# phymhan/pc-gan

Measured on AMD Instinct MI355X. Metric: images/sec (G+D step) 128x128 bs32 per GPU, higher is better.
Workload: dtype f32; 1 GPU; wsgan_emb UTKFace-shaped 128x128 bs32/GPU fp32: 9-block ResnetGenerator + 3-layer PatchGAN + ResNet-18 Elo encoder@224 + AlexNet IP@224, full optimize_parameters(); global_batch=32, parallelism=dp1

## Files before the change

include/pcgan_hip.h:

```cpp
#ifndef PCGAN_HIP_H
#define PCGAN_HIP_H

#include <stddef.h>
#include <stdint.h>

#ifdef __cplusplus
extern "C" {
#endif

typedef void* pcgan_stream_t;

const char* pcgan_last_error(void);
int pcgan_version(void);
int pcgan_device_info(int* cu_count, char* arch, int arch_len);

typedef struct {
    int N, C, H, W;
    int K, R, S;
    int stride, pad, pad_mode;
    int P, Q;
    int dtype;
} pcgan_conv_desc;

enum { PCGAN_ACT_NONE = 0, PCGAN_ACT_RELU = 1, PCGAN_ACT_LRELU = 2, PCGAN_ACT_TANH = 3, PCGAN_ACT_SIGMOID = 4 };
// ... 46 lines not shown
                         int act, float slope, int dtype, pcgan_stream_t s);
int pcgan_bn_bwd_reduce(const float* s1_nc, const float* s2_nc, float* s1_c, float* s2_c, int N, int C,
                        pcgan_stream_t s);
int pcgan_bn_stats_merged(const void* x, float* mean_nc, float* m2_nc, float* mean_c, float* var_c, float* running_mean,
                          float* running_var, long long* batches, unsigned int* ticket, int N, int C, int HW, float momentum, int dtype,
                          pcgan_stream_t s);
int pcgan_bn_bwd_stats_reduced(const void* dy, const void* x, const void* y, const float* mean_c, const float* var_c, float* s1_nc,
                               float* s2_nc, float* s1_c, float* s2_c, unsigned int* ticket, int N, int C, int HW, float eps, int act,
                               float slope, int dtype, pcgan_stream_t s);
int pcgan_bn_fwd_fused(const void* x, const float* gamma, const float* beta, const void* residual, void* y,
                       float* mean_c, float* var_c, float* running_mean, float* running_var, long long* batches, float* y_cmax,
                       int N, int C, int HW, float momentum, float eps, int act, float slope, int dtype, pcgan_stream_t s);
int pcgan_bn_bwd_fused(const void* dy, const void* x, const void* y, const float* mean_c, const float* var_c,
                       const float* gamma, void* dx, void* dres, float* s1_c, float* s2_c, float* dx_cmax, int N, int C, int HW,
                       float eps, int act, float slope, int dtype, pcgan_stream_t s);

int pcgan_instnorm_fwd(const void* x, const void* residual, void* y, float* mean_nc, float* m2_nc, float* y_pmax, int N, int C,
                       int HW, float eps, int act, float slope, int dtype, pcgan_stream_t s);
int pcgan_instnorm_bwd(const void* dy, const void* x, const void* y, const float* mean_nc, const float* m2_nc,
                       void* dx, float* dx_psum, float* dx_pmax, float* ws_s1s2, int N, int C, int HW, float eps, int act,
                       float slope, int dtype, pcgan_stream_t s);
int pcgan_instnorm_fused(int HW);
int pcgan_sum_planes(const float* part_nc, float* out, int N, int C, int accumulate, pcgan_stream_t s);

int pcgan_maxpool_fwd(const void* x, void* y, int32_t* argmax, int NC, int H, int W, int k, int stride,
                      int pad, int P, int Q, int dtype, pcgan_stream_t s);
int pcgan_maxpool_bwd(const void* dy, const int32_t* argmax, void* dx, int NC, int H, int W, int k, int stride,
                      int pad, int P, int Q, int dtype, pcgan_stream_t s);
int pcgan_avgpool_fwd(const void* x, void* y, int NC, int H, int W, int k, int stride, int pad, int P, int Q, int dtype,
                      pcgan_stream_t s);
// ... 223 lines not shown
```

pc-gan_amd/csrc/capi.hip:

```cpp
#include "common.h"
#include <stdarg.h>
#include <atomic>
#include <mutex>
#include <vector>

namespace pcgan {
static thread_local char g_err[512] = "";
void set_error(const char* fmt, ...) {
    va_list ap;
    va_start(ap, fmt);
    vsnprintf(g_err, sizeof(g_err), fmt, ap);
    va_end(ap);
}
}

namespace pcgan {
namespace {
struct TimerKind {
    std::vector<hipEvent_t> start, stop;
    int used = 0;
};
std::mutex g_timer_mu;
std::atomic<int> g_timer_on{0};
TimerKind g_timer[TIMER_KINDS];
// ... 57 lines not shown
    }
    t.used = 0;
    return n;
}

namespace pcgan {
static std::atomic<unsigned*> g_nonfinite{nullptr};
unsigned* nonfinite_counter() { return g_nonfinite.load(std::memory_order_relaxed); }
}
extern "C" int pcgan_set_nonfinite_counter(unsigned int* dev_word) {
    pcgan::g_nonfinite.store(dev_word);
    return 0;
}

namespace pcgan {
static const char* const g_opt_names[OPT_COUNT] = {"bsplit_halo", "wgrad_gen", "wgrad_padcopy", "wgrad_cw", "hgemm_bf16", "wgd_look", "wgrad_direct", "hgemm_tile", "hgemm_ks", "wgrad_rowring", "wgrad_ks", "hwgrad_ks"};
static std::atomic<int> g_opt[OPT_COUNT] = {{1}, {1}, {0}, {0}, {1}, {3}, {0}, {0}, {0}, {1}, {0}, {0}};
int option(int id) { return (id >= 0 && id < OPT_COUNT) ? g_opt[id].load(std::memory_order_relaxed) : 0; }
static int option_index(const char* key) {
    for (int i = 0; key && i < OPT_COUNT; ++i)
        if (strcmp(key, g_opt_names[i]) == 0) return i;
    return -1;
}
}
extern "C" int pcgan_set_option(const char* key, int value) {
    using namespace pcgan;
    const int i = option_index(key);
    PCGAN_CHECK(i >= 0, "set_option: unknown option '%s' (bsplit_halo, wgrad_gen, wgrad_padcopy, wgrad_cw, hgemm_bf16, wgd_look, wgrad_direct, hgemm_tile, hgemm_ks, wgrad_rowring, wgrad_ks, hwgrad_ks)", key ? key : "(null)");
    PCGAN_CHECK(i != OPT_WGRAD_CW || value == 0 || value == 128 || value == 256, "set_option: wgrad_cw takes 0 (default), 128 or 256, got %d", value);
    PCGAN_CHECK(i != OPT_HGEMM_TILE || value == 0 || value == 128128 || value == 128064 || value == 64128 || value == 64064,
                "set_option: hgemm_tile takes 0 (heuristic) or BM * 1000 + BP with BM, BP in {64, 128}, got %d", value);
    PCGAN_CHECK(i != OPT_HGEMM_KS || (value >= 0 && value <= 8), "set_option: hgemm_ks takes 0 (heuristic) .. 8, got %d", value);
    PCGAN_CHECK(i != OPT_WGRAD_KS || (value >= 0 && value <= 512), "set_option: wgrad_ks takes 0 (heuristic) .. 512, got %d", value);
    PCGAN_CHECK(i != OPT_HWGRAD_KS || (value >= 0 && value <= 512), "set_option: hwgrad_ks takes 0 (heuristic) .. 512, got %d", value);
    g_opt[i].store(value);
    return 0;
}
extern "C" int pcgan_get_option(const char* key, int* value) {
    using namespace pcgan;
    const int i = option_index(key);
    PCGAN_CHECK(i >= 0 && value, "get_option: unknown option or null output");
    *value = g_opt[i].load();
    return 0;
}

extern "C" const char* pcgan_last_error(void) { return pcgan::g_err; }
extern "C" int pcgan_version(void) { return 100; }

extern "C" int pcgan_device_info(int* cu_count, char* arch, int arch_len) {
// ... 14 lines not shown
```

pc-gan_amd/csrc/common.h:

```cpp
#pragma once
#include <hip/hip_runtime.h>
#include <stdint.h>
#include <stdio.h>
#include <string.h>
#include "../../include/pcgan_hip.h"

namespace pcgan {

void set_error(const char* fmt, ...);

#define PCGAN_CHECK(cond, ...)                \
    do {                                      \
        if (!(cond)) {                        \
            pcgan::set_error(__VA_ARGS__);    \
            return 1;                         \
        }                                     \
    } while (0)

#define PCGAN_LAUNCH_CHECK()                                                      \
    do {                                                                          \
        hipError_t e__ = hipGetLastError();                                       \
        if (e__ != hipSuccess) {                                                  \
            pcgan::set_error("%s:%d launch failed: %s", __FILE__, __LINE__,       \
                             hipGetErrorString(e__));                             \
// ... 1 lines not shown
        }                                                                         \
    } while (0)

enum { TIMER_RES_FWD = 0, TIMER_RES_DGRAD = 1, TIMER_RES_WGRAD = 2, TIMER_RES_WGRAD_MAIN = 3, TIMER_KINDS = 4 };
struct TimerScope {
    int kind, slot;
    hipStream_t st;
    TimerScope(int kind, hipStream_t st);
    ~TimerScope();
};

static inline int timer_kind_res(const pcgan_conv_desc* d, int kind) {
    return (d && d->K == 256 && d->C == 256 && d->R == 3 && d->S == 3 && d->stride == 1 && d->pad_mode == 1 && d->pad == 1) ? kind : -1;
}

enum { OPT_BSPLIT_HALO = 0, OPT_WGRAD_GEN = 1, OPT_WGRAD_PADCOPY = 2, OPT_WGRAD_CW = 3, OPT_HGEMM_BF16 = 4, OPT_WGD_LOOK = 5, OPT_WGRAD_DIRECT = 6, OPT_HGEMM_TILE = 7, OPT_HGEMM_KS = 8, OPT_WGRAD_ROWRING = 9, OPT_WGRAD_KS = 10, OPT_HWGRAD_KS = 11, OPT_COUNT = 12 };
int option(int id);

unsigned* nonfinite_counter();
int launch_wgd_reduce(const float* part, float* dw, const float* scales, int splits, int K, int C, int accumulate, hipStream_t st);
__device__ __forceinline__ bool is_nonfinite(float v) { return (__float_as_uint(v) & 0x7f800000u) == 0x7f800000u; }
__device__ __forceinline__ void report_nonfinite(unsigned* counter, bool bad) {
    if (counter != nullptr && __builtin_amdgcn_ballot_w64(bad) != 0ull && (threadIdx.x & 63) == 0) atomicAdd(counter, 1u);
}

int launch_weight_row_absmax(const float* w, int K, int C, int T, int by_c, float* out, hipStream_t st);

int launch_reflect_fold(const void* padded, void* dx, int NC, int H, int W, int pad, int dtype, hipStream_t st, const float* bias = nullptr,
                        int C = 1);

static inline int ilog2_exact(int v) {
// ... 176 lines not shown
```

pc-gan_amd/csrc/norm.hip:

```cpp
#include <type_traits>

#include "common.h"

namespace pcgan {

struct BnTicket {
    unsigned* ticket;
    int N, C;
};
template <bool WT>
__device__ __forceinline__ void bn_merge_channel(const float* mean_nc, const float* m2_nc, float* __restrict__ mean_c,
                                                 float* __restrict__ var_c, float* running_mean, float* running_var, int N, int C, int HW,
                                                 float momentum, int c, int lane) {
    float msum = 0.f;
    for (int n = lane; n < N; n += 64) msum += WT ? ld_wt(mean_nc + n * C + c) : mean_nc[n * C + c];
    const float mean = wave_sum(msum) / (float)N;
    float m2 = 0.f;
    for (int n = lane; n < N; n += 64) {
        const float d = (WT ? ld_wt(mean_nc + n * C + c) : mean_nc[n * C + c]) - mean;
        m2 += (WT ? ld_wt(m2_nc + n * C + c) : m2_nc[n * C + c]) + d * d * (float)HW;
    }
    m2 = wave_sum(m2);
    if (lane != 0) return;
    const float cnt = (float)N * (float)HW;
// ... 48 lines not shown
template <int V, bool SQ, typename T>
__device__ __forceinline__ float plane_partial(const T* xp, int n, float mean) {
    float s = 0.f;
    for (int i = threadIdx.x; i < n; i += blockDim.x) {
        float v[V];
        ldv<V>(xp + V * i, v);
        if (SQ) {
#pragma unroll
            for (int e = 0; e < V; ++e) v[e] = (v[e] - mean) * (v[e] - mean);
        }
        s += vsum<V>(v);
    }
    return s;
}

template <typename T>
__global__ void __launch_bounds__(256) plane_stats_kernel(const T* __restrict__ x, float* __restrict__ mean_nc,
                                                          float* __restrict__ m2_nc, int HW, BnTicket tk = BnTicket{nullptr, 0, 0},
                                                          BnMergeOut mo = BnMergeOut{nullptr, nullptr, nullptr, nullptr, nullptr, 0.f}) {
    __shared__ float scratch[16];
    const size_t plane = blockIdx.x;
    const T* xp = x + plane * (size_t)HW;
    const bool v4 = (HW & 3) == 0;
    const float s = v4 ? plane_partial<4, false>(xp, HW >> 2, 0.f) : plane_partial<1, false>(xp, HW, 0.f);
    const float mean = block_sum(s, scratch) / (float)HW;
    const float q = v4 ? plane_partial<4, true>(xp, HW >> 2, mean) : plane_partial<1, true>(xp, HW, mean);
    const float m2 = block_sum(q, scratch);
    if (threadIdx.x == 0) {
        if (tk.ticket != nullptr) {
            st_wt(mean_nc + plane, mean);
            st_wt(m2_nc + plane, m2);
        } else {
            mean_nc[plane] = mean;
            m2_nc[plane] = m2;
        }
    }
    if (tk.ticket != nullptr) {
        __shared__ int last_flag;
        const int c = (int)(plane % (size_t)tk.C);
        if (block_arrives_last(tk.ticket, c, (unsigned)tk.N, &last_flag) && threadIdx.x < 64) {
            bn_merge_channel<true>(mean_nc, m2_nc, mo.mean_c, mo.var_c, mo.running_mean, mo.running_var, tk.N, tk.C, HW, mo.momentum, c, threadIdx.x);
            if (c == 0 && threadIdx.x == 0 && mo.batches) mo.batches[0] += 1;
// ... 84 lines not shown
    const size_t plane = blockIdx.x;
    float mean, rstd, g, b;
    plane_coeffs(a, plane, mean, rstd, g, b);
    const float sc = rstd * g, sh = b - mean * rstd * g;
    const T* xp = (const T*)a.x + plane * (size_t)a.HW;
    const T* rp = a.residual ? (const T*)a.residual + plane * (size_t)a.HW : nullptr;
    T* yp = (T*)a.out + plane * (size_t)a.HW;
    float am = (a.HW & 3) == 0 ? norm_act_plane<4>(a, xp, rp, yp, a.HW >> 2, sc, sh) : norm_act_plane<1>(a, xp, rp, yp, a.HW, sc, sh);
    if (a.pmax) {
        __shared__ float scratch[16];
        am = block_max(am, scratch);
        if (threadIdx.x == 0) a.pmax[plane] = am;
    }
}

template <typename T>
__global__ void __launch_bounds__(256) norm_bwd_stats_kernel(NormArgs a, BnTicket tk = BnTicket{nullptr, 0, 0}, float* s1_c = nullptr,
                                                             float* s2_c = nullptr) {
    __shared__ float scratch[16];
    const size_t plane = blockIdx.x;
    float mean, rstd, g_, b_;
    plane_coeffs(a, plane, mean, rstd, g_, b_);
    const T* xp = (const T*)a.x + plane * (size_t)a.HW;
    const T* dp = (const T*)a.dy + plane * (size_t)a.HW;
    const T* yp = (a.act != PCGAN_ACT_NONE) ? (const T*)a.y + plane * (size_t)a.HW : nullptr;
    float s1 = 0.f, s2 = 0.f;
    for (int i = threadIdx.x; i < a.HW; i += blockDim.x) {
        float g = ld1(dp + i);
        if (yp) g *= act_grad_from_out(ld1(yp + i), a.act, a.slope);
        s1 += g;
        s2 += g * ((ld1(xp + i) - mean) * rstd);
    }
    s1 = block_sum(s1, scratch);
    s2 = block_sum(s2, scratch);
    if (threadIdx.x == 0) {
        if (tk.ticket != nullptr) {
            st_wt((float*)a.out + plane, s1);
            st_wt((float*)a.out2 + plane, s2);
        } else {
            ((float*)a.out)[plane] = s1;
            ((float*)a.out2)[plane] = s2;
        }
    }
    if (tk.ticket != nullptr) {
        __shared__ int last_flag;
        const int c = (int)(plane % (size_t)tk.C);
// ... 150 lines not shown
            float g = d[e];
            if (act != PCGAN_ACT_NONE) g *= act_grad_from_out(yv[e], act, slope);
            gr[e] = g;
            o[e] = kk * (g - m1 - ((xv[e] - mean) * rstd) * m2);
            am = fmaxf(am, fabsf(o[e]));
        }
        if (dx) stv<V>(dx + i, o);
        if (dres) stv<V>(dres + i, gr);
    });
    if (dx && dx_cmax) {
        am = block_max(am, scratch);
        if (threadIdx.x == 0) dx_cmax[c] = am;
    }
}

struct PlaneBlock {
    float* scratch;
    __device__ __forceinline__ int first() const { return threadIdx.x; }
    __device__ __forceinline__ int step() const { return blockDim.x; }
    __device__ __forceinline__ float sum(float v) const { return block_sum(v, scratch); }
    __device__ __forceinline__ float max(float v) const { return block_max(v, scratch); }
};
struct PlaneWave {
    int lane;
    __device__ __forceinline__ int first() const { return lane; }
    __device__ __forceinline__ int step() const { return 64; }
    __device__ __forceinline__ float sum(float v) const { return wave_sum(v); }
    __device__ __forceinline__ float max(float v) const { return wave_max(v); }
};

// ... 214 lines not shown
    static constexpr bool wave = W;
    static constexpr int E = E_;
};
template <typename F>
static void instnorm_dispatch(int E, int NT, int planes, F launch) {
    if (E == 1 && planes >= 1024) launch(InstnormForm<true, 4>{}, dim3((planes + 3) / 4), dim3(256));
    else if (E == 1) launch(InstnormForm<false, 1>{}, dim3(planes), dim3(NT));
    else if (E == 4) launch(InstnormForm<false, 4>{}, dim3(planes), dim3(NT));
    else launch(InstnormForm<false, 16>{}, dim3(planes), dim3(NT));
}
template <typename F>
static void bn_fused_dispatch(int HW, F launch) {
    if ((HW & 3) == 0) launch(std::integral_constant<int, 4>{});
    else launch(std::integral_constant<int, 1>{});
}

}

using namespace pcgan;

extern "C" int pcgan_plane_stats(const void* x, float* mean_nc, float* m2_nc, int NC, int HW, int dtype, pcgan_stream_t s) {
    PCGAN_CHECK(x && mean_nc && m2_nc && NC > 0 && HW > 0, "plane_stats: bad arguments");
    PCGAN_DTYPE_SWITCH(dtype, T, hipLaunchKernelGGL(plane_stats_kernel<T>, dim3(NC), dim3(plane_threads(HW)), 0, (hipStream_t)s,
                                                    (const T*)x, mean_nc, m2_nc, HW));
    PCGAN_LAUNCH_CHECK();
    return 0;
}

extern "C" int pcgan_bn_stats_merged(const void* x, float* mean_nc, float* m2_nc, float* mean_c, float* var_c, float* running_mean,
                                     float* running_var, long long* batches, unsigned int* ticket, int N, int C, int HW, float momentum,
                                     int dtype, pcgan_stream_t s) {
    PCGAN_CHECK(x && mean_nc && m2_nc && mean_c && var_c && ticket && N > 0 && C > 0 && HW > 0 && (long long)N * HW > 1, "bn_stats_merged: bad arguments");
    const BnTicket tk{ticket, N, C};
    const BnMergeOut mo{mean_c, var_c, running_mean, running_var, batches, momentum};
    PCGAN_DTYPE_SWITCH(dtype, T, hipLaunchKernelGGL(plane_stats_kernel<T>, dim3(N * C), dim3(plane_threads(HW)), 0, (hipStream_t)s,
                                                    (const T*)x, mean_nc, m2_nc, HW, tk, mo));
    PCGAN_LAUNCH_CHECK();
    return 0;
}

extern "C" int pcgan_bn_bwd_stats_reduced(const void* dy, const void* x, const void* y, const float* mean_c, const float* var_c, float* s1_nc,
                                          float* s2_nc, float* s1_c, float* s2_c, unsigned int* ticket, int N, int C, int HW, float eps, int act,
                                          float slope, int dtype, pcgan_stream_t s) {
    PCGAN_CHECK(dy && x && mean_c && var_c && s1_nc && s2_nc && s1_c && s2_c && ticket && N > 0 && C > 0 && HW > 0, "bn_bwd_stats_reduced: bad arguments");
    PCGAN_CHECK(act == PCGAN_ACT_NONE || y, "bn_bwd_stats_reduced: activation mask needs y");
    NormArgs a = norm_args(x, mean_c, var_c, N, C, HW, 0, eps, act, slope);
    a.y = y; a.dy = dy; a.out = s1_nc; a.out2 = s2_nc;
    const BnTicket tk{ticket, N, C};
    PCGAN_DTYPE_SWITCH(dtype, T, hipLaunchKernelGGL(norm_bwd_stats_kernel<T>, dim3(N * C), dim3(plane_threads(HW)), 0, (hipStream_t)s, a, tk, s1_c, s2_c));
    PCGAN_LAUNCH_CHECK();
    return 0;
}

extern "C" int pcgan_bn_merge(const float* mean_nc, const float* m2_nc, float* mean_c, float* var_c,
                              float* running_mean, float* running_var, int N, int C, int HW, float momentum,
                              pcgan_stream_t s) {
    PCGAN_CHECK(mean_nc && m2_nc && N > 0 && C > 0 && HW > 0, "bn_merge: bad arguments");
    hipLaunchKernelGGL(bn_merge_kernel, dim3((C + 3) / 4), dim3(256), 0, (hipStream_t)s, mean_nc, m2_nc, mean_c,
                       var_c, running_mean, running_var, N, C, HW, momentum);
    PCGAN_LAUNCH_CHECK();
    return 0;
}

extern "C" int pcgan_in_running_update(const float* mean_nc, const float* m2_nc, float* running_mean,
// ... 13 lines not shown
    PCGAN_CHECK(x && mean && var && y && N > 0 && C > 0 && HW > 0, "norm_act_fwd: bad arguments");
    NormArgs a = norm_args(x, mean, var, N, C, HW, per_plane, eps, act, slope);
    a.gamma = gamma; a.beta = beta; a.residual = residual; a.out = y; a.pmax = y_pmax;
    PCGAN_DTYPE_SWITCH(dtype, T, hipLaunchKernelGGL(norm_act_fwd_kernel<T>, dim3(N * C), dim3(plane_threads(HW)), 0, (hipStream_t)s, a));
    PCGAN_LAUNCH_CHECK();
    return 0;
}

extern "C" int pcgan_norm_bwd_stats(const void* dy, const void* x, const void* y, const float* mean,
                                    const float* var, float* s1_nc, float* s2_nc, int N, int C, int HW,
                                    int per_plane, float eps, int act, float slope, int dtype, pcgan_stream_t s) {
    PCGAN_CHECK(dy && x && mean && var && s1_nc && s2_nc, "norm_bwd_stats: null pointer");
    PCGAN_CHECK(act == PCGAN_ACT_NONE || y, "norm_bwd_stats: activation mask needs y");
    NormArgs a = norm_args(x, mean, var, N, C, HW, per_plane, eps, act, slope);
    a.y = y; a.dy = dy; a.out = s1_nc; a.out2 = s2_nc;
    PCGAN_DTYPE_SWITCH(dtype, T, hipLaunchKernelGGL(norm_bwd_stats_kernel<T>, dim3(N * C), dim3(plane_threads(HW)), 0, (hipStream_t)s, a));
    PCGAN_LAUNCH_CHECK();
    return 0;
}

extern "C" int pcgan_bn_bwd_reduce(const float* s1_nc, const float* s2_nc, float* s1_c, float* s2_c, int N, int C,
                                   pcgan_stream_t s) {
    PCGAN_CHECK(s1_nc && s2_nc && s1_c && s2_c, "bn_bwd_reduce: null pointer");
    hipLaunchKernelGGL(bn_bwd_reduce_kernel, dim3((C + 3) / 4), dim3(256), 0, (hipStream_t)s, s1_nc, s2_nc, s1_c,
                       s2_c, N, C);
    PCGAN_LAUNCH_CHECK();
    return 0;
}

extern "C" int pcgan_norm_bwd_apply(const void* dy, const void* x, const void* y, const float* mean,
                                    const float* var, const float* gamma, const float* s1, const float* s2,
// ... 73 lines not shown
        if (pcgan_norm_bwd_stats(dy, x, y, mean_nc, m2_nc, ws_s1s2, ws_s1s2 + (size_t)N * C, N, C, HW, 1, eps, act, slope, dtype, s))
            return 1;
        return pcgan_norm_bwd_apply(dy, x, y, mean_nc, m2_nc, nullptr, ws_s1s2, ws_s1s2 + (size_t)N * C, dx, nullptr, nullptr, N, C,
                                    HW, 1, eps, act, slope, dtype, s);
    }
    PCGAN_DTYPE_SWITCH(dtype, T, launch_instnorm_bwd<T>(E, NT, N * C, st, dy, x, y, mean_nc, m2_nc, dx, dx_psum, HW, eps, act, slope, dx_pmax));
    PCGAN_LAUNCH_CHECK();
    return 0;
}

template <typename T>
static void launch_bn_fwd(hipStream_t st, const void* x, const float* gamma, const float* beta, const void* residual, void* y,
                          float* mean_c, float* var_c, float* running_mean, float* running_var, long long* batches, int N, int C, int HW,
                          float momentum, float eps, int act, float slope, float* y_cmax) {
    bn_fused_dispatch(HW, [&](auto v) {
        hipLaunchKernelGGL((bn_fwd_fused_kernel<decltype(v)::value, T>), dim3(C), dim3(256), 0, st, (const T*)x, gamma, beta, (const T*)residual, (T*)y,
                           mean_c, var_c, running_mean, running_var, batches, N, C, HW, momentum, eps, act, slope, y_cmax);
    });
}

extern "C" int pcgan_bn_fwd_fused(const void* x, const float* gamma, const float* beta, const void* residual, void* y,
                                  float* mean_c, float* var_c, float* running_mean, float* running_var, long long* batches,
                                  float* y_cmax, int N, int C, int HW, float momentum, float eps, int act, float slope, int dtype,
                                  pcgan_stream_t s) {
    PCGAN_CHECK(x && y && mean_c && var_c && N > 0 && C > 0 && HW > 0 && (long long)N * HW > 1, "bn_fwd_fused: bad arguments");
    PCGAN_DTYPE_SWITCH(dtype, T, launch_bn_fwd<T>((hipStream_t)s, x, gamma, beta, residual, y, mean_c, var_c, running_mean,
                                                  running_var, batches, N, C, HW, momentum, eps, act, slope, y_cmax));
    PCGAN_LAUNCH_CHECK();
    return 0;
}

template <typename T>
static void launch_bn_bwd(hipStream_t st, const void* dy, const void* x, const void* y, const float* mean_c, const float* var_c,
                          const float* gamma, void* dx, void* dres, float* s1_c, float* s2_c, int N, int C, int HW, float eps, int act, float slope,
                          float* dx_cmax) {
    bn_fused_dispatch(HW, [&](auto v) {
        hipLaunchKernelGGL((bn_bwd_fused_kernel<decltype(v)::value, T>), dim3(C), dim3(256), 0, st, (const T*)dy, (const T*)x, (const T*)y, mean_c, var_c,
                           gamma, (T*)dx, (T*)dres, s1_c, s2_c, N, C, HW, eps, act, slope, dx_cmax);
    });
}

extern "C" int pcgan_bn_bwd_fused(const void* dy, const void* x, const void* y, const float* mean_c, const float* var_c,
                                  const float* gamma, void* dx, void* dres, float* s1_c, float* s2_c, float* dx_cmax, int N, int C, int HW,
                                  float eps, int act, float slope, int dtype, pcgan_stream_t s) {
    PCGAN_CHECK(dy && x && mean_c && var_c && s1_c && s2_c && N > 0 && C > 0 && HW > 0, "bn_bwd_fused: bad arguments");
    PCGAN_CHECK(act == PCGAN_ACT_NONE || y, "bn_bwd_fused: activation mask needs y");
    PCGAN_DTYPE_SWITCH(dtype, T, launch_bn_bwd<T>((hipStream_t)s, dy, x, y, mean_c, var_c, gamma, dx, dres, s1_c, s2_c, N, C, HW,
                                                  eps, act, slope, dx_cmax));
    PCGAN_LAUNCH_CHECK();
    return 0;
}
```

pc-gan_amd/hip/lib.py:

```python
import ctypes
import os

_HERE = os.path.dirname(os.path.abspath(__file__))
LIB_PATH = os.environ.get('PCGAN_LIB') or os.path.join(os.path.dirname(_HERE), 'lib', 'libpcgan_hip.so')

ACT_NONE, ACT_RELU, ACT_LRELU, ACT_TANH, ACT_SIGMOID = 0, 1, 2, 3, 4
PASS_FWD, PASS_BWD_DATA, PASS_BWD_WEIGHT = 0, 1, 2
F32, BF16 = 0, 1
ADD_N_MAX = 8
POOL_PLAN_MAX = 64
GCAM_TYPES = {'raw': 0, 'pw': 1, 'cw_pos': 2, 'pw_cw': 3}
POOL_PASS = -1


def pool_store(s):
    return 2 * int(s)


def pool_swap(s):
    return 2 * int(s) + 1


def pool_exchange_launches():
    return int(load().pcgan_pool_exchange_launches())
# ... 43 lines not shown
    'pcgan_add': (_i, [_vp, _vp, _vp, _sz, _i, _vp]),
    'pcgan_scale': (_i, [_vp, _vp, _f, _vp, _sz, _i, _vp]),
    'pcgan_cast': (_i, [_vp, _i, _vp, _i, _sz, _vp]),
    'pcgan_channel_scale': (_i, [_vp, _vp, _vp, _i, _i, _f, _i, _vp]),
    'pcgan_plane_stats': (_i, [_vp, _vp, _vp, _i, _i, _i, _vp]),
    'pcgan_bn_merge': (_i, [_vp, _vp, _vp, _vp, _vp, _vp, _i, _i, _i, _f, _vp]),
    'pcgan_in_running_update': (_i, [_vp, _vp, _vp, _vp, _i, _i, _i, _f, _vp]),
    'pcgan_norm_act_fwd': (_i, [_vp, _vp, _vp, _vp, _vp, _vp, _vp, _vp, _i, _i, _i, _i, _f, _i, _f, _i, _vp]),
    'pcgan_norm_bwd_stats': (_i, [_vp, _vp, _vp, _vp, _vp, _vp, _vp, _i, _i, _i, _i, _f, _i, _f, _i, _vp]),
    'pcgan_norm_bwd_apply': (_i, [_vp, _vp, _vp, _vp, _vp, _vp, _vp, _vp, _vp, _vp, _vp, _i, _i, _i, _i, _f, _i, _f, _i, _vp]),
    'pcgan_bn_bwd_reduce': (_i, [_vp, _vp, _vp, _vp, _i, _i, _vp]),
    'pcgan_bn_stats_merged': (_i, [_vp, _vp, _vp, _vp, _vp, _vp, _vp, _vp, _vp, _i, _i, _i, _f, _i, _vp]),
    'pcgan_bn_bwd_stats_reduced': (_i, [_vp, _vp, _vp, _vp, _vp, _vp, _vp, _vp, _vp, _vp, _i, _i, _i, _f, _i, _f, _i, _vp]),
    'pcgan_bn_fwd_fused': (_i, [_vp, _vp, _vp, _vp, _vp, _vp, _vp, _vp, _vp, _vp, _vp, _i, _i, _i, _f, _f, _i, _f, _i, _vp]),
    'pcgan_bn_bwd_fused': (_i, [_vp, _vp, _vp, _vp, _vp, _vp, _vp, _vp, _vp, _vp, _vp, _i, _i, _i, _f, _i, _f, _i, _vp]),
    'pcgan_instnorm_fwd': (_i, [_vp, _vp, _vp, _vp, _vp, _vp, _i, _i, _i, _f, _i, _f, _i, _vp]),
    'pcgan_instnorm_bwd': (_i, [_vp, _vp, _vp, _vp, _vp, _vp, _vp, _vp, _vp, _i, _i, _i, _f, _i, _f, _i, _vp]),
    'pcgan_instnorm_fused': (_i, [_i]),
    'pcgan_sum_planes': (_i, [_vp, _vp, _i, _i, _i, _vp]),
    'pcgan_maxpool_fwd': (_i, [_vp, _vp, _vp, _i, _i, _i, _i, _i, _i, _i, _i, _i, _vp]),
    'pcgan_maxpool_bwd': (_i, [_vp, _vp, _vp, _i, _i, _i, _i, _i, _i, _i, _i, _i, _vp]),
    'pcgan_avgpool_fwd': (_i, [_vp, _vp, _i, _i, _i, _i, _i, _i, _i, _i, _i, _vp]),
    'pcgan_avgpool_bwd': (_i, [_vp, _vp, _vp, _i, _i, _i, _i, _i, _i, _i, _i, _i, _vp]),
    'pcgan_global_pool_fwd': (_i, [_vp, _vp, _vp, _i, _i, _i, _i, _vp]),
    'pcgan_global_pool_bwd': (_i, [_vp, _vp, _vp, _i, _i, _i, _i, _vp]),
    'pcgan_bilinear_fwd': (_i, [_vp, _vp, _i, _i, _i, _i, _i, _i, _vp]),
    'pcgan_bilinear_bwd': (_i, [_vp, _vp, _i, _i, _i, _i, _i, _i, _vp]),
    'pcgan_bce_loss': (_i, [_vp, _vp, _vp, _vp, _i, _i, _f, _vp, _sz, _i, _vp]),
    'pcgan_l1_loss': (_i, [_vp, _vp, _vp, _vp, _sz, _f, _vp, _sz, _i, _vp]),
    'pcgan_mse_loss': (_i, [_vp, _vp, _vp, _vp, _sz, _f, _vp, _sz, _i, _vp]),
# ... 102 lines not shown
    bundled = os.path.join(os.path.dirname(torch.__file__), 'lib', 'libamdhip64.so')
    if os.path.exists(bundled):
        ctypes.CDLL(bundled, mode=ctypes.RTLD_GLOBAL)
    lib = ctypes.CDLL(LIB_PATH)
    for name, (res, args) in SIGNATURES.items():
        fn = getattr(lib, name)
        fn.restype = res
        fn.argtypes = args
    _lib = lib
    _options_from_environment(lib)
    return lib


_ENV_OPTIONS = (('PCGAN_BSPLIT_HALO', 'bsplit_halo', int), ('PCGAN_WGRAD_GEN', 'wgrad_gen', int), ('PCGAN_WGRAD_PADCOPY', 'wgrad_padcopy', int),
                ('PCGAN_WGRAD_CW', 'wgrad_cw', int), ('PCGAN_HGEMM', 'hgemm_bf16', int), ('PCGAN_WGRAD_DIRECT', 'wgrad_direct', int),
                ('PCGAN_WGD_LOOK', 'wgd_look', int), ('PCGAN_WGRAD_ROWRING', 'wgrad_rowring', int))


def _options_from_environment(lib):
    for env, key, conv in _ENV_OPTIONS:
        v = os.environ.get(env)
        if v not in (None, ''):
            set_option(key, conv(v), lib)


def set_option(key, value, lib=None):
    lib = lib or load()
    if lib.pcgan_set_option(key.encode(), int(value)) != 0:
        msg = lib.pcgan_last_error()
        raise RuntimeError('pcgan_hip set_option failed: %s' % (msg.decode() if msg else '?'))

# ... 13 lines not shown
```

Measured before the change: 1168 images/sec.

## Keep normalization tiles register-resident to avoid re-reading inputs across passes

```diff
diff --git a/include/pcgan_hip.h b/include/pcgan_hip.h
--- a/include/pcgan_hip.h
+++ b/include/pcgan_hip.h
@@ -84,6 +84,7 @@
 int pcgan_bn_bwd_fused(const void* dy, const void* x, const void* y, const float* mean_c, const float* var_c,
                        const float* gamma, void* dx, void* dres, float* s1_c, float* s2_c, float* dx_cmax, int N, int C, int HW,
                        float eps, int act, float slope, int dtype, pcgan_stream_t s);
+int pcgan_bn_resident_bound(int kind, int N, int HW);
 
 int pcgan_instnorm_fwd(const void* x, const void* residual, void* y, float* mean_nc, float* m2_nc, float* y_pmax, int N, int C,
                        int HW, float eps, int act, float slope, int dtype, pcgan_stream_t s);
diff --git a/pc-gan_amd/csrc/capi.hip b/pc-gan_amd/csrc/capi.hip
--- a/pc-gan_amd/csrc/capi.hip
+++ b/pc-gan_amd/csrc/capi.hip
@@ -95,8 +95,8 @@
 }
 
 namespace pcgan {
-static const char* const g_opt_names[OPT_COUNT] = {"bsplit_halo", "wgrad_gen", "wgrad_padcopy", "wgrad_cw", "hgemm_bf16", "wgd_look", "wgrad_direct", "hgemm_tile", "hgemm_ks", "wgrad_rowring", "wgrad_ks", "hwgrad_ks"};
-static std::atomic<int> g_opt[OPT_COUNT] = {{1}, {1}, {0}, {0}, {1}, {3}, {0}, {0}, {0}, {1}, {0}, {0}};
+static const char* const g_opt_names[OPT_COUNT] = {"bsplit_halo", "wgrad_gen", "wgrad_padcopy", "wgrad_cw", "hgemm_bf16", "wgd_look", "wgrad_direct", "hgemm_tile", "hgemm_ks", "wgrad_rowring", "wgrad_ks", "hwgrad_ks", "bn_resident"};
+static std::atomic<int> g_opt[OPT_COUNT] = {{1}, {1}, {0}, {0}, {1}, {3}, {0}, {0}, {0}, {1}, {0}, {0}, {1}};
 int option(int id) { return (id >= 0 && id < OPT_COUNT) ? g_opt[id].load(std::memory_order_relaxed) : 0; }
 static int option_index(const char* key) {
     for (int i = 0; key && i < OPT_COUNT; ++i)
@@ -107,13 +107,14 @@
 extern "C" int pcgan_set_option(const char* key, int value) {
     using namespace pcgan;
     const int i = option_index(key);
-    PCGAN_CHECK(i >= 0, "set_option: unknown option '%s' (bsplit_halo, wgrad_gen, wgrad_padcopy, wgrad_cw, hgemm_bf16, wgd_look, wgrad_direct, hgemm_tile, hgemm_ks, wgrad_rowring, wgrad_ks, hwgrad_ks)", key ? key : "(null)");
+    PCGAN_CHECK(i >= 0, "set_option: unknown option '%s' (bsplit_halo, wgrad_gen, wgrad_padcopy, wgrad_cw, hgemm_bf16, wgd_look, wgrad_direct, hgemm_tile, hgemm_ks, wgrad_rowring, wgrad_ks, hwgrad_ks, bn_resident)", key ? key : "(null)");
     PCGAN_CHECK(i != OPT_WGRAD_CW || value == 0 || value == 128 || value == 256, "set_option: wgrad_cw takes 0 (default), 128 or 256, got %d", value);
     PCGAN_CHECK(i != OPT_HGEMM_TILE || value == 0 || value == 128128 || value == 128064 || value == 64128 || value == 64064,
                 "set_option: hgemm_tile takes 0 (heuristic) or BM * 1000 + BP with BM, BP in {64, 128}, got %d", value);
     PCGAN_CHECK(i != OPT_HGEMM_KS || (value >= 0 && value <= 8), "set_option: hgemm_ks takes 0 (heuristic) .. 8, got %d", value);
     PCGAN_CHECK(i != OPT_WGRAD_KS || (value >= 0 && value <= 512), "set_option: wgrad_ks takes 0 (heuristic) .. 512, got %d", value);
     PCGAN_CHECK(i != OPT_HWGRAD_KS || (value >= 0 && value <= 512), "set_option: hwgrad_ks takes 0 (heuristic) .. 512, got %d", value);
+    PCGAN_CHECK(i != OPT_BN_RESIDENT || value == 0 || value == 1, "set_option: bn_resident takes 0 or 1, got %d", value);
     g_opt[i].store(value);
     return 0;
 }
diff --git a/pc-gan_amd/csrc/common.h b/pc-gan_amd/csrc/common.h
--- a/pc-gan_amd/csrc/common.h
+++ b/pc-gan_amd/csrc/common.h
@@ -39,7 +39,7 @@
     return (d && d->K == 256 && d->C == 256 && d->R == 3 && d->S == 3 && d->stride == 1 && d->pad_mode == 1 && d->pad == 1) ? kind : -1;
 }
 
-enum { OPT_BSPLIT_HALO = 0, OPT_WGRAD_GEN = 1, OPT_WGRAD_PADCOPY = 2, OPT_WGRAD_CW = 3, OPT_HGEMM_BF16 = 4, OPT_WGD_LOOK = 5, OPT_WGRAD_DIRECT = 6, OPT_HGEMM_TILE = 7, OPT_HGEMM_KS = 8, OPT_WGRAD_ROWRING = 9, OPT_WGRAD_KS = 10, OPT_HWGRAD_KS = 11, OPT_COUNT = 12 };
+enum { OPT_BSPLIT_HALO = 0, OPT_WGRAD_GEN = 1, OPT_WGRAD_PADCOPY = 2, OPT_WGRAD_CW = 3, OPT_HGEMM_BF16 = 4, OPT_WGD_LOOK = 5, OPT_WGRAD_DIRECT = 6, OPT_HGEMM_TILE = 7, OPT_HGEMM_KS = 8, OPT_WGRAD_ROWRING = 9, OPT_WGRAD_KS = 10, OPT_HWGRAD_KS = 11, OPT_BN_RESIDENT = 12, OPT_COUNT = 13 };
 int option(int id);
 
 unsigned* nonfinite_counter();
diff --git a/pc-gan_amd/csrc/norm.hip b/pc-gan_amd/csrc/norm.hip
--- a/pc-gan_amd/csrc/norm.hip
+++ b/pc-gan_amd/csrc/norm.hip
@@ -86,7 +86,39 @@
     return s;
 }
 
-template <typename T>
+template <int V, int G, typename T>
+__device__ __forceinline__ void plane_stats_resident(const T* xp, int n, int HW, float* scratch, float& mean, float& m2) {
+    float v[G][V];
+#pragma unroll
+    for (int k = 0; k < G; ++k) {
+        const int i = threadIdx.x + k * blockDim.x;
+        ldv<V>(xp + V * (i < n ? i : n - 1), v[k]);
+    }
+    float s = 0.f;
+#pragma unroll
+    for (int k = 0; k < G; ++k)
+        if ((int)(threadIdx.x + k * blockDim.x) < n) s += vsum<V>(v[k]);
+    mean = block_sum(s, scratch) / (float)HW;
+    float q = 0.f;
+#pragma unroll
+    for (int k = 0; k < G; ++k) {
+#pragma clang fp contract(off)
+        float d[V];
+#pragma unroll
+        for (int e = 0; e < V; ++e) d[e] = v[k][e] - mean;
+        const bool ok = (int)(threadIdx.x + k * blockDim.x) < n;
+        if (V == 4) {
+            const float t = __builtin_fmaf(d[0], d[0], d[1 % V] * d[1 % V]) + __builtin_fmaf(d[2 % V], d[2 % V], d[3 % V] * d[3 % V]);
+            if (ok) q += t;
+        } else if (ok) {
+            q = __builtin_fmaf(d[0], d[0], q);
+        }
+    }
+    m2 = block_sum(q, scratch);
+}
+constexpr int PLANE_RESIDENT_GROUPS = 16;
+
+template <typename T, int G>
 __global__ void __launch_bounds__(256) plane_stats_kernel(const T* __restrict__ x, float* __restrict__ mean_nc,
                                                           float* __restrict__ m2_nc, int HW, BnTicket tk = BnTicket{nullptr, 0, 0},
                                                           BnMergeOut mo = BnMergeOut{nullptr, nullptr, nullptr, nullptr, nullptr, 0.f}) {
@@ -94,10 +126,16 @@
     const size_t plane = blockIdx.x;
     const T* xp = x + plane * (size_t)HW;
     const bool v4 = (HW & 3) == 0;
-    const float s = v4 ? plane_partial<4, false>(xp, HW >> 2, 0.f) : plane_partial<1, false>(xp, HW, 0.f);
-    const float mean = block_sum(s, scratch) / (float)HW;
-    const float q = v4 ? plane_partial<4, true>(xp, HW >> 2, mean) : plane_partial<1, true>(xp, HW, mean);
-    const float m2 = block_sum(q, scratch);
+    float mean, m2;
+    if constexpr (G > 0) {
+        if (v4) plane_stats_resident<4, G>(xp, HW >> 2, HW, scratch, mean, m2);
+        else plane_stats_resident<1, G>(xp, HW, HW, scratch, mean, m2);
+    } else {
+        const float s = v4 ? plane_partial<4, false>(xp, HW >> 2, 0.f) : plane_partial<1, false>(xp, HW, 0.f);
+        mean = block_sum(s, scratch) / (float)HW;
+        const float q = v4 ? plane_partial<4, true>(xp, HW >> 2, mean) : plane_partial<1, true>(xp, HW, mean);
+        m2 = block_sum(q, scratch);
+    }
     if (threadIdx.x == 0) {
         if (tk.ticket != nullptr) {
             st_wt(mean_nc + plane, mean);
@@ -212,7 +250,7 @@
     }
 }
 
-template <typename T>
+template <typename T, int G>
 __global__ void __launch_bounds__(256) norm_bwd_stats_kernel(NormArgs a, BnTicket tk = BnTicket{nullptr, 0, 0}, float* s1_c = nullptr,
                                                              float* s2_c = nullptr) {
     __shared__ float scratch[16];
@@ -223,11 +261,38 @@
     const T* dp = (const T*)a.dy + plane * (size_t)a.HW;
     const T* yp = (a.act != PCGAN_ACT_NONE) ? (const T*)a.y + plane * (size_t)a.HW : nullptr;
     float s1 = 0.f, s2 = 0.f;
-    for (int i = threadIdx.x; i < a.HW; i += blockDim.x) {
-        float g = ld1(dp + i);
-        if (yp) g *= act_grad_from_out(ld1(yp + i), a.act, a.slope);
-        s1 += g;
-        s2 += g * ((ld1(xp + i) - mean) * rstd);
+    if constexpr (G > 0) {
+        float d[G], xv[G], yv[G];
+#pragma unroll
+        for (int k = 0; k < G; ++k) {
+            const int i = threadIdx.x + k * blockDim.x, ic = i < a.HW ? i : a.HW - 1;
+            d[k] = ld1(dp + ic);
+            xv[k] = ld1(xp + ic);
+        }
+        if (yp) {
+#pragma unroll
+            for (int k = 0; k < G; ++k) {
+                const int i = threadIdx.x + k * blockDim.x;
+                yv[k] = ld1(yp + (i < a.HW ? i : a.HW - 1));
+            }
+        }
+#pragma unroll
+        for (int k = 0; k < G; ++k) {
+#pragma clang fp contract(off)
+            float g = d[k];
+            if (yp) g *= act_grad_from_out(yv[k], a.act, a.slope);
+            if ((int)(threadIdx.x + k * blockDim.x) < a.HW) {
+                s1 += g;
+                s2 += g * ((xv[k] - mean) * rstd);
+            }
+        }
+    } else {
+        for (int i = threadIdx.x; i < a.HW; i += blockDim.x) {
+            float g = ld1(dp + i);
+            if (yp) g *= act_grad_from_out(ld1(yp + i), a.act, a.slope);
+            s1 += g;
+            s2 += g * ((ld1(xp + i) - mean) * rstd);
+        }
     }
     s1 = block_sum(s1, scratch);
     s2 = block_sum(s2, scratch);
@@ -408,6 +473,165 @@
     }
 }
 
+template <int V, int G>
+struct BnGroups {
+    unsigned own;
+    int C, HW, c, KG;
+    __device__ __forceinline__ BnGroups(int N, int C_, int HW_, int c_, int KG_) : own(0u), C(C_), HW(HW_), c(c_), KG(KG_) {
+        const int ln = threadIdx.x & 63;
+        int n = threadIdx.x >> 6, kk = 0;
+#pragma unroll
+        for (int g = 0; g < G; ++g) {
+            if (n < N && (kk * 64 + ln) * V < HW) own |= 1u << g;
+            if (++kk == KG) { kk = 0; n += 4; }
+        }
+    }
+    template <typename F>
+    __device__ __forceinline__ void each(F f) const {
+        const int ln = threadIdx.x & 63;
+        int n = threadIdx.x >> 6, kk = 0;
+#pragma unroll
+        for (int g = 0; g < G; ++g) {
+            const bool owned = (own >> g) & 1u;
+            f(g, owned, owned ? ((size_t)n * C + c) * HW + (size_t)((kk * 64 + ln) * V) : (size_t)c * HW);
+            if (++kk == KG) { kk = 0; n += 4; }
+        }
+    }
+};
+
+template <int V, int G, typename T>
+__global__ void __launch_bounds__(256, 2) bn_fwd_resident_kernel(const T* __restrict__ x, const float* __restrict__ gamma,
+                                                                 const float* __restrict__ beta, const T* __restrict__ res,
+                                                                 T* __restrict__ y, float* __restrict__ mean_c,
+                                                                 float* __restrict__ var_c, float* running_mean, float* running_var,
+                                                                 long long* batches, int N, int C, int HW, int KG, float momentum, float eps,
+                                                                 int act, float slope, float* __restrict__ y_cmax) {
+#pragma clang fp contract(off)
+    __shared__ float scratch[16];
+    const int c = blockIdx.x;
+    const int cnt = N * HW;
+    const BnGroups<V, G> grp(N, C, HW, c, KG);
+    constexpr bool RES_EARLY = G * V <= 64;
+    float v[G][V], r[RES_EARLY ? G : 1][V];
+    grp.each([&](int g, bool, size_t i) { ldv<V>(x + i, v[g]); });
+    if (RES_EARLY && res) grp.each([&](int g, bool, size_t i) { ldv<V>(res + i, r[RES_EARLY ? g : 0]); });
+    float s = 0.f;
+    grp.each([&](int g, bool owned, size_t) {
+        if (owned) {
+#pragma unroll
+            for (int e = 0; e < V; ++e) s += v[g][e];
+        }
+    });
+    const float mean = block_sum(s, scratch) / (float)cnt;
+    float q = 0.f;
+    grp.each([&](int g, bool owned, size_t) {
+        if (owned) {
+#pragma unroll
+            for (int e = 0; e < V; ++e) {
+                const float d = v[g][e] - mean;
+                q = V == 1 ? __builtin_fmaf(d, d, q) : q + d * d;
+            }
+        }
+    });
+    const float m2 = block_sum(q, scratch);
+    const float var = m2 / (float)cnt;
+    if (threadIdx.x == 0) {
+        mean_c[c] = mean;
+        var_c[c] = var;
+        if (running_mean) running_mean[c] = (1.f - momentum) * running_mean[c] + momentum * mean;
+        if (running_var) running_var[c] = (1.f - momentum) * running_var[c] + momentum * (m2 / ((float)cnt - 1.f));
+        if (batches && c == 0) batches[0] += 1;
+    }
+    const float ga = gamma ? gamma[c] : 1.f, b = beta ? beta[c] : 0.f;
+    const float sc = rsqrtf(var + eps) * ga, sh = __builtin_fmaf(-mean, sc, b);
+    float am = 0.f;
+    grp.each([&](int g, bool owned, size_t i) {
+        float rl[V];
+        if (!RES_EARLY && res) ldv<V>(res + i, rl);
+#pragma unroll
+        for (int e = 0; e < V; ++e) {
+            float t = __builtin_fmaf(v[g][e], sc, sh);
+            if (res) t += RES_EARLY ? r[RES_EARLY ? g : 0][e] : rl[e];
+            v[g][e] = act_apply(t, act, slope);
+            if (owned) am = fmaxf(am, fabsf(v[g][e]));
+        }
+        if (owned) stv<V>(y + i, v[g]);
+    });
+    if (y_cmax) {
+        am = block_max(am, scratch);
+        if (threadIdx.x == 0) y_cmax[c] = am;
+    }
+}
+
+template <int V, int G, typename T>
+__global__ void __launch_bounds__(256, 2) bn_bwd_resident_kernel(const T* __restrict__ dy, const T* __restrict__ x,
+                                                                 const T* __restrict__ y, const float* __restrict__ mean_c,
+                                                                 const float* __restrict__ var_c, const float* __restrict__ gamma,
+                                                                 T* __restrict__ dx, T* __restrict__ dres,
+                                                                 float* __restrict__ s1_c, float* __restrict__ s2_c, int N, int C,
+                                                                 int HW, int KG, float eps, int act, float slope, float* __restrict__ dx_cmax) {
+#pragma clang fp contract(off)
+    __shared__ float scratch[16];
+    const int c = blockIdx.x;
+    const int cnt = N * HW;
+    const BnGroups<V, G> grp(N, C, HW, c, KG);
+    constexpr bool Y_EARLY = G * V <= 32;
+    float gr[G][V], xh[G][V], yv[Y_EARLY ? G : 1][V];
+    const bool masked = act != PCGAN_ACT_NONE;
+    grp.each([&](int g, bool, size_t i) { ldv<V>(dy + i, gr[g]); });
+    if (Y_EARLY) {
+        grp.each([&](int g, bool, size_t i) { ldv<V>(x + i, xh[g]); });
+        if (masked) grp.each([&](int g, bool, size_t i) { ldv<V>(y + i, yv[Y_EARLY ? g : 0]); });
+    } else if (masked) {
+        grp.each([&](int g, bool, size_t i) { ldv<V>(y + i, xh[g]); });
+    }
+    const float mean = mean_c[c], rstd = rsqrtf(var_c[c] + eps);
+    if (masked) {
+        grp.each([&](int g, bool, size_t) {
+#pragma unroll
+            for (int e = 0; e < V; ++e) gr[g][e] *= act_grad_from_out(Y_EARLY ? yv[Y_EARLY ? g : 0][e] : xh[g][e], act, slope);
+        });
+    }
+    if (!Y_EARLY) grp.each([&](int g, bool, size_t i) { ldv<V>(x + i, xh[g]); });
+    float s1 = 0.f, s2 = 0.f;
+    grp.each([&](int g, bool owned, size_t) {
+#pragma unroll
+        for (int e = 0; e < V; ++e) {
+            xh[g][e] = (xh[g][e] - mean) * rstd;
+            if (owned) {
+                s1 += gr[g][e];
+                s2 += gr[g][e] * xh[g][e];
+            }
+        }
+    });
+    s1 = block_sum(s1, scratch);
+    s2 = block_sum(s2, scratch);
+    if (threadIdx.x == 0) {
+        s1_c[c] = s1;
+        s2_c[c] = s2;
+    }
+    if (!dx && !dres) return;
+    const float m1 = s1 / (float)cnt, m2 = s2 / (float)cnt;
+    const float kk = rstd * (gamma ? gamma[c] : 1.f);
+    float am = 0.f;
+    grp.each([&](int g, bool owned, size_t i) {
+        float o[V];
+#pragma unroll
+        for (int e = 0; e < V; ++e) {
+            o[e] = kk * __builtin_fmaf(-xh[g][e], m2, gr[g][e] - m1);
+            if (owned) am = fmaxf(am, fabsf(o[e]));
+        }
+        if (owned) {
+            if (dx) stv<V>(dx + i, o);
+            if (dres) stv<V>(dres + i, gr[g]);
+        }
+    });
+    if (dx && dx_cmax) {
+        am = block_max(am, scratch);
+        if (threadIdx.x == 0) dx_cmax[c] = am;
+    }
+}
+
 struct PlaneBlock {
     float* scratch;
     __device__ __forceinline__ int first() const { return threadIdx.x; }
@@ -652,6 +876,23 @@
     if ((HW & 3) == 0) launch(std::integral_constant<int, 4>{});
     else launch(std::integral_constant<int, 1>{});
 }
+static int bn_resident_bound(int N, int HW, bool backward) {
+    if (!option(OPT_BN_RESIDENT)) return 0;
+    const int V = (HW & 3) == 0 ? 4 : 1;
+    const long long groups = (long long)((N + 3) / 4) * ((HW + 64 * V - 1) / (64 * V));
+    if (groups > ((backward && V == 4) ? 16 : 32)) return 0;
+    return groups <= 8 ? 8 : (groups <= 16 ? 16 : 32);
+}
+static int plane_resident_bound(int HW, bool vectorised) {
+    if (!option(OPT_BN_RESIDENT)) return 0;
+    const int n = (vectorised && (HW & 3) == 0) ? HW >> 2 : HW;
+    return (long long)n <= (long long)PLANE_RESIDENT_GROUPS * plane_threads(HW) ? PLANE_RESIDENT_GROUPS : 0;
+}
+template <int... Gs, typename F>
+static void resident_dispatch(int bound, F launch) {
+    const bool hit = ((bound == Gs ? (launch(std::integral_constant<int, Gs>{}), true) : false) || ...);
+    if (!hit) launch(std::integral_constant<int, 0>{});
+}
 
 }
 
@@ -659,8 +900,10 @@
 
 extern "C" int pcgan_plane_stats(const void* x, float* mean_nc, float* m2_nc, int NC, int HW, int dtype, pcgan_stream_t s) {
     PCGAN_CHECK(x && mean_nc && m2_nc && NC > 0 && HW > 0, "plane_stats: bad arguments");
-    PCGAN_DTYPE_SWITCH(dtype, T, hipLaunchKernelGGL(plane_stats_kernel<T>, dim3(NC), dim3(plane_threads(HW)), 0, (hipStream_t)s,
-                                                    (const T*)x, mean_nc, m2_nc, HW));
+    PCGAN_DTYPE_SWITCH(dtype, T, resident_dispatch<PLANE_RESIDENT_GROUPS>(plane_resident_bound(HW, true), [&](auto g) {
+        hipLaunchKernelGGL((plane_stats_kernel<T, decltype(g)::value>), dim3(NC), dim3(plane_threads(HW)), 0, (hipStream_t)s, (const T*)x, mean_nc,
+                           m2_nc, HW, BnTicket{nullptr, 0, 0}, BnMergeOut{nullptr, nullptr, nullptr, nullptr, nullptr, 0.f});
+    }));
     PCGAN_LAUNCH_CHECK();
     return 0;
 }
@@ -671,8 +914,10 @@
     PCGAN_CHECK(x && mean_nc && m2_nc && mean_c && var_c && ticket && N > 0 && C > 0 && HW > 0 && (long long)N * HW > 1, "bn_stats_merged: bad arguments");
     const BnTicket tk{ticket, N, C};
     const BnMergeOut mo{mean_c, var_c, running_mean, running_var, batches, momentum};
-    PCGAN_DTYPE_SWITCH(dtype, T, hipLaunchKernelGGL(plane_stats_kernel<T>, dim3(N * C), dim3(plane_threads(HW)), 0, (hipStream_t)s,
-                                                    (const T*)x, mean_nc, m2_nc, HW, tk, mo));
+    PCGAN_DTYPE_SWITCH(dtype, T, resident_dispatch<PLANE_RESIDENT_GROUPS>(plane_resident_bound(HW, true), [&](auto g) {
+        hipLaunchKernelGGL((plane_stats_kernel<T, decltype(g)::value>), dim3(N * C), dim3(plane_threads(HW)), 0, (hipStream_t)s, (const T*)x,
+                           mean_nc, m2_nc, HW, tk, mo);
+    }));
     PCGAN_LAUNCH_CHECK();
     return 0;
 }
@@ -685,7 +930,9 @@
     NormArgs a = norm_args(x, mean_c, var_c, N, C, HW, 0, eps, act, slope);
     a.y = y; a.dy = dy; a.out = s1_nc; a.out2 = s2_nc;
     const BnTicket tk{ticket, N, C};
-    PCGAN_DTYPE_SWITCH(dtype, T, hipLaunchKernelGGL(norm_bwd_stats_kernel<T>, dim3(N * C), dim3(plane_threads(HW)), 0, (hipStream_t)s, a, tk, s1_c, s2_c));
+    PCGAN_DTYPE_SWITCH(dtype, T, resident_dispatch<PLANE_RESIDENT_GROUPS>(plane_resident_bound(HW, false), [&](auto g) {
+        hipLaunchKernelGGL((norm_bwd_stats_kernel<T, decltype(g)::value>), dim3(N * C), dim3(plane_threads(HW)), 0, (hipStream_t)s, a, tk, s1_c, s2_c);
+    }));
     PCGAN_LAUNCH_CHECK();
     return 0;
 }
@@ -729,7 +976,10 @@
     PCGAN_CHECK(act == PCGAN_ACT_NONE || y, "norm_bwd_stats: activation mask needs y");
     NormArgs a = norm_args(x, mean, var, N, C, HW, per_plane, eps, act, slope);
     a.y = y; a.dy = dy; a.out = s1_nc; a.out2 = s2_nc;
-    PCGAN_DTYPE_SWITCH(dtype, T, hipLaunchKernelGGL(norm_bwd_stats_kernel<T>, dim3(N * C), dim3(plane_threads(HW)), 0, (hipStream_t)s, a));
+    PCGAN_DTYPE_SWITCH(dtype, T, resident_dispatch<PLANE_RESIDENT_GROUPS>(plane_resident_bound(HW, false), [&](auto g) {
+        hipLaunchKernelGGL((norm_bwd_stats_kernel<T, decltype(g)::value>), dim3(N * C), dim3(plane_threads(HW)), 0, (hipStream_t)s, a,
+                           BnTicket{nullptr, 0, 0}, (float*)nullptr, (float*)nullptr);
+    }));
     PCGAN_LAUNCH_CHECK();
     return 0;
 }
@@ -833,8 +1083,17 @@
                           float* mean_c, float* var_c, float* running_mean, float* running_var, long long* batches, int N, int C, int HW,
                           float momentum, float eps, int act, float slope, float* y_cmax) {
     bn_fused_dispatch(HW, [&](auto v) {
-        hipLaunchKernelGGL((bn_fwd_fused_kernel<decltype(v)::value, T>), dim3(C), dim3(256), 0, st, (const T*)x, gamma, beta, (const T*)residual, (T*)y,
-                           mean_c, var_c, running_mean, running_var, batches, N, C, HW, momentum, eps, act, slope, y_cmax);
+        constexpr int V = decltype(v)::value;
+        resident_dispatch<8, 16, 32>(bn_resident_bound(N, HW, false), [&](auto g) {
+            constexpr int G = decltype(g)::value;
+            if constexpr (G > 0)
+                hipLaunchKernelGGL((bn_fwd_resident_kernel<V, G, T>), dim3(C), dim3(256), 0, st, (const T*)x, gamma, beta, (const T*)residual, (T*)y,
+                                   mean_c, var_c, running_mean, running_var, batches, N, C, HW, (HW + 64 * V - 1) / (64 * V), momentum, eps, act,
+                                   slope, y_cmax);
+            else
+                hipLaunchKernelGGL((bn_fwd_fused_kernel<V, T>), dim3(C), dim3(256), 0, st, (const T*)x, gamma, beta, (const T*)residual, (T*)y,
+                                   mean_c, var_c, running_mean, running_var, batches, N, C, HW, momentum, eps, act, slope, y_cmax);
+        });
     });
 }
 
@@ -854,9 +1113,25 @@
                           const float* gamma, void* dx, void* dres, float* s1_c, float* s2_c, int N, int C, int HW, float eps, int act, float slope,
                           float* dx_cmax) {
     bn_fused_dispatch(HW, [&](auto v) {
-        hipLaunchKernelGGL((bn_bwd_fused_kernel<decltype(v)::value, T>), dim3(C), dim3(256), 0, st, (const T*)dy, (const T*)x, (const T*)y, mean_c, var_c,
-                           gamma, (T*)dx, (T*)dres, s1_c, s2_c, N, C, HW, eps, act, slope, dx_cmax);
-    });
+        constexpr int V = decltype(v)::value;
+        resident_dispatch<8, 16, 32>(bn_resident_bound(N, HW, true), [&](auto g) {
+            constexpr int G = decltype(g)::value;
+            if constexpr (G > 0 && G * V <= 64)
+                hipLaunchKernelGGL((bn_bwd_resident_kernel<V, G, T>), dim3(C), dim3(256), 0, st, (const T*)dy, (const T*)x, (const T*)y, mean_c, var_c,
+                                   gamma, (T*)dx, (T*)dres, s1_c, s2_c, N, C, HW, (HW + 64 * V - 1) / (64 * V), eps, act, slope, dx_cmax);
+            else
+                hipLaunchKernelGGL((bn_bwd_fused_kernel<V, T>), dim3(C), dim3(256), 0, st, (const T*)dy, (const T*)x, (const T*)y, mean_c, var_c,
+                                   gamma, (T*)dx, (T*)dres, s1_c, s2_c, N, C, HW, eps, act, slope, dx_cmax);
+        });
+    });
+}
+
+extern "C" int pcgan_bn_resident_bound(int kind, int N, int HW) {
+    if (kind < 0 || kind > 3 || N <= 0 || HW <= 0) {
+        pcgan::set_error("bn_resident_bound: kind 0 .. 3, N > 0, HW > 0");
+        return -1;
+    }
+    return kind <= 1 ? bn_resident_bound(N, HW, kind == 1) : plane_resident_bound(HW, kind == 2);
 }
 
 extern "C" int pcgan_bn_bwd_fused(const void* dy, const void* x, const void* y, const float* mean_c, const float* var_c,
diff --git a/pc-gan_amd/hip/lib.py b/pc-gan_amd/hip/lib.py
--- a/pc-gan_amd/hip/lib.py
+++ b/pc-gan_amd/hip/lib.py
@@ -81,6 +81,7 @@
     'pcgan_bn_bwd_stats_reduced': (_i, [_vp, _vp, _vp, _vp, _vp, _vp, _vp, _vp, _vp, _vp, _i, _i, _i, _f, _i, _f, _i, _vp]),
     'pcgan_bn_fwd_fused': (_i, [_vp, _vp, _vp, _vp, _vp, _vp, _vp, _vp, _vp, _vp, _vp, _i, _i, _i, _f, _f, _i, _f, _i, _vp]),
     'pcgan_bn_bwd_fused': (_i, [_vp, _vp, _vp, _vp, _vp, _vp, _vp, _vp, _vp, _vp, _vp, _i, _i, _i, _f, _i, _f, _i, _vp]),
+    'pcgan_bn_resident_bound': (_i, [_i, _i, _i]),
     'pcgan_instnorm_fwd': (_i, [_vp, _vp, _vp, _vp, _vp, _vp, _i, _i, _i, _f, _i, _f, _i, _vp]),
     'pcgan_instnorm_bwd': (_i, [_vp, _vp, _vp, _vp, _vp, _vp, _vp, _vp, _vp, _i, _i, _i, _f, _i, _f, _i, _vp]),
     'pcgan_instnorm_fused': (_i, [_i]),
@@ -213,7 +214,7 @@
 
 _ENV_OPTIONS = (('PCGAN_BSPLIT_HALO', 'bsplit_halo', int), ('PCGAN_WGRAD_GEN', 'wgrad_gen', int), ('PCGAN_WGRAD_PADCOPY', 'wgrad_padcopy', int),
                 ('PCGAN_WGRAD_CW', 'wgrad_cw', int), ('PCGAN_HGEMM', 'hgemm_bf16', int), ('PCGAN_WGRAD_DIRECT', 'wgrad_direct', int),
-                ('PCGAN_WGD_LOOK', 'wgd_look', int), ('PCGAN_WGRAD_ROWRING', 'wgrad_rowring', int))
+                ('PCGAN_WGD_LOOK', 'wgd_look', int), ('PCGAN_WGRAD_ROWRING', 'wgrad_rowring', int), ('PCGAN_BN_RESIDENT', 'bn_resident', int))
 
 
 def _options_from_environment(lib):
```

Result: no change. 1161 images/sec (-0.6%).
